# ikt-luh/Unified-Point-Cloud-Compression

Hardware: AMD Instinct MI355X
Metric: points/sec encode+decode, longdress vox10, 1 GPU; bpp & D1-PSNR parity (higher is better)
Workload: dtype f32

## Files before the change

### include/pcc_hip.h

```cpp
#ifndef PCC_HIP_H
#define PCC_HIP_H

#include <stddef.h>
#include <stdint.h>

#ifdef __cplusplus
extern "C" {
#endif

#define PCC_OK 0
#define PCC_EINVAL (-1)
#define PCC_EHIP (-2)
#define PCC_EWS (-3)

#define PCC_ACT_NONE 0
#define PCC_ACT_RELU 1
#define PCC_ACT_LEAKY 2

#define PCC_MAP_HDR_INTS 512
#define PCC_MAP_MAX_SEG 8

int pcc_version(void);
const char* pcc_last_error(void);
int pcc_device_info(int* h_cu_count, char* h_arch, int h_arch_len);
// ... 80 lines not shown
int pcc_set_in4_min_rows(int64_t rows);
int pcc_set_thin_z_min_rows(int64_t rows);
int64_t pcc_conv_packed_elems(int32_t K, int32_t cin, int32_t cout);
int pcc_conv_pack_weights(const float* W, int32_t K, int32_t cin, int32_t cout, float* packed,
                          int64_t packed_cap, void* stream);
int pcc_conv_pack_weights_ex(const float* W, int32_t K, int32_t cin, int32_t cout, int32_t transpose, int32_t flip, float* packed,
                             int64_t packed_cap, void* stream);
size_t pcc_conv_ws_bytes(int64_t n_in, int32_t K, int32_t cin, int32_t cout);
int pcc_conv_head_supported(int32_t cin, int32_t cmid);
size_t pcc_conv_head_ws_bytes(int64_t n);
int pcc_conv_head_fwd(const float* feat, int64_t n, int32_t cin, const float* packed_w0, const float* bias0 ,
                      int32_t cmid, const float* w2, const float* bias2 , const int32_t* hdr,
                      const int32_t* nbr, const int32_t* tiles, const int32_t* n_tiles, float* logits, void* ws,
                      size_t ws_bytes, void* stream);
int64_t pcc_band_tiles_cap(int64_t n, int32_t nx, int32_t nbands);
size_t pcc_band_tiles_ws_bytes(int32_t nx, int32_t nbands);
int pcc_band_tiles_build(const int64_t* keys, int64_t n, int32_t lo_x, int32_t nx, int32_t lo_y, int32_t ny, int32_t ts,
                         int32_t nbands, int32_t* tiles, int64_t tiles_cap, int32_t* n_tiles , void* ws,
                         size_t ws_bytes, void* stream);
int pcc_conv_fwd(const float* feat_in, int64_t n_in, int32_t cin, const float* packed_w,
                 const float* bias , int32_t K, int32_t cout, const int32_t* hdr,
                 const int32_t* nbr, const int32_t* rows, int64_t n_out, float* out, int32_t act,
                 float slope, void* ws, size_t ws_bytes, int32_t arith, int32_t* d_guard , void* stream);
int pcc_conv_pairs_supported(int32_t K, int32_t cin, int32_t cout);
size_t pcc_pair_plan_ws_bytes(int64_t n_out, int32_t K);
int pcc_pair_plan_rank(const int32_t* nbr, int64_t n_out, int32_t K, int32_t* pos, int32_t* pstart, int64_t* info,
                       void* ws, size_t ws_bytes, void* stream);
int pcc_pair_plan_fill(const int32_t* nbr, const int32_t* pos, const int32_t* pstart, int64_t n_out, int32_t K,
                       int64_t padded_pairs, int32_t* pair_in, int32_t* tile_k, void* stream);
int pcc_conv_fwd_pairs(const float* feat_in, int64_t n_in, int32_t cin, const float* packed_w, const float* bias,
                       int32_t K, int32_t cout, const int32_t* pair_in, const int32_t* tile_k, const int64_t* d_info,
                       int64_t padded_pairs, const int32_t* pos, int64_t n_out, float* T, float* out, int32_t act,
                       float slope, int32_t arith, int32_t* d_guard , void* stream);


int64_t pcc_convt_packed_elems(int32_t K, int32_t cin, int32_t cout);
int pcc_convt_pack_weights(const float* W, int32_t K, int32_t cin, int32_t cout, float* packed,
                           int64_t packed_cap, void* stream);
int pcc_convt_fwd(const float* feat_in, int64_t n_in, int32_t cin, const float* packed_w,
                  const float* bias , int32_t K, int32_t cout, const int32_t* hdr,
                  const int32_t* nbr, const int32_t* rows, int64_t n_out, float* T, float* out, int32_t act,
                  float slope, int32_t arith, int32_t* d_guard , void* stream);

int pcc_convt_fwd_csr(const float* feat_in, int64_t n_in, int32_t cin, const float* packed_w,
                      const float* bias , int32_t K, int32_t cout, const int32_t* first,
                      const int32_t* pair_ids, int64_t n_out, float* T, float* out, int32_t act, float slope,
                      const int32_t* ex_nbr , int32_t ex_K,
                      const float* ex_bias , int32_t arith, int32_t* d_guard , void* stream);

int pcc_convt_fwd_csr_grid(const float* feat_in, int64_t n_in, int32_t cin, const float* packed_w, const float* bias ,
                           int32_t K, int32_t cout, const int32_t* first, const int32_t* pair_ids, int64_t n_out, float* T,
                           float* out, int32_t act, float slope, const int64_t* out_keys, const uint64_t* out_bits,
                           const int32_t* out_rank, const int32_t* h_out, const float* ex_bias,
                           const int32_t* wg_end ,
                           int32_t arith, int32_t* d_guard , void* stream);
size_t pcc_thin_grid_ws_bytes(int64_t n, int32_t cout);
int pcc_conv_thin_grid_fwd(const float* feat, int64_t n, int32_t cin, const float* packed_w, const float* bias ,
                           int32_t cout, const int64_t* keys, const uint64_t* bits, const int32_t* rank, const int32_t* h_grid,
                           float* out, void* ws, size_t ws_bytes, void* stream);

int64_t pcc_gdn_packed_elems(int32_t c);
int pcc_gdn_pack(const float* beta_raw, const float* gamma_raw, int32_t c, float beta_min,
                 float* packed, int64_t packed_cap, float* beta_eff, void* stream);
int pcc_gdn_fwd(const float* x, int64_t n, int32_t c, const float* packed, const float* beta_eff,
                int32_t inverse, float* out, int32_t arith, void* stream);

// ... 161 lines not shown
```

### unified_point_cloud_compression_amd/autograd.py

```python

import torch

from . import lib as L
from . import sparse as S


GDN_FUSED_BWD = True
WGRAD_SELF = True


def _pack(w3):
    p = S.PackedConv()
    return p.get(w3.contiguous())


def _pad4(t, dim):
    r = (-t.shape[dim]) % 4
    if r == 0:
        return t
    shape = list(t.shape)
    shape[dim] = r
    return torch.cat([t, t.new_zeros(shape)], dim=dim)


def _pack_view(src3, K, cin, cout, transpose, flip):
    src3 = src3.contiguous()
    n = L.load().pcc_conv_packed_elems(K, cin, cout)
    packed = torch.empty(n, dtype=torch.float32, device=src3.device)
    L.call("pcc_conv_pack_weights_ex", L.ptr(src3), K, cin, cout, 1 if transpose else 0, 1 if flip else 0, L.ptr(packed),
           packed.numel(), L.stream())
    return packed


def _conv_view(feats, src3, transpose, flip, kmap, n_out):
    K, a, b = src3.shape
    cin, cout = (b, a) if transpose else (a, b)
    if cin % 32 == 0 and cout > 16 and feats.shape[1] == cin:
        return S.conv_forward(feats, _pack_view(src3, K, cin, cout, transpose, flip), None, K, cin, cout, kmap, n_out)
    w = torch.flip(src3, dims=[0]) if flip else src3
    return _conv_any(feats, w.permute(0, 2, 1) if transpose else w, kmap, n_out)


def _conv_any(feats, w3, kmap, n_out):
    K, cin, cout = w3.shape
    if cin % 4 != 0:
        feats, w3 = _pad4(feats, 1), _pad4(w3, 1)
        cin = w3.shape[1]
    if cin > 16 and cin % 32 != 0:
        r = (-cin) % 32
        feats = torch.cat([feats, feats.new_zeros((feats.shape[0], r))], dim=1)
        w3 = torch.cat([w3, w3.new_zeros((K, r, cout))], dim=1)
        cin += r
    if cin not in (4, 8, 16) and cin % 32 != 0:
        r = 16 - cin
        feats = torch.cat([feats, feats.new_zeros((feats.shape[0], r))], dim=1)
        w3 = torch.cat([w3, w3.new_zeros((K, r, cout))], dim=1)
        cin = 16
    return S.conv_forward(feats, _pack(w3), None, K, cin, cout, kmap, n_out)


class SparseConvFn(torch.autograd.Function):

    @staticmethod
    def forward(ctx, feats, kernel, bias, module, in_set, out_set, kmap, act, slope):
        K, cin, cout = module.kernel_volume, module.in_channels, module.out_channels
        packed = module._packed.get(kernel, tag_from=module.kernel)
        feats = feats.contiguous()
        if isinstance(kmap, tuple):
            out = S.convt_forward_csr(feats, packed, bias, K, cin, cout, kmap, out_set.n, act, slope)
        elif module.TRANSPOSED:
            out = S.convt_forward(feats, packed, bias, K, cin, cout, kmap, out_set.n, act, slope)
        else:
            out = S.conv_forward(feats, packed, bias, K, cin, cout, kmap, out_set.n, act, slope)
        ctx.save_for_backward(feats, kernel, out if act != L.ACT_NONE else None)
        ctx.meta = (module, in_set, out_set, kmap, act, slope, bias is not None)
        return out

    @staticmethod
    def backward(ctx, g):
        feats, kernel, out = ctx.saved_tensors
        module, in_set, out_set, kmap, act, slope, has_bias = ctx.meta
        K, cin, cout = module.kernel_volume, module.in_channels, module.out_channels
        g = g.contiguous()
        if act == L.ACT_RELU:
            g = g * (out > 0)
        elif act == L.ACT_LEAKY:
            g = torch.where(out > 0, g, g * slope)
        w3 = kernel.detach() if kernel.dim() == 3 else kernel.detach().unsqueeze(0)
        g_feats = g_kernel = g_bias = None
        if has_bias and ctx.needs_input_grad[2]:
            g_bias = g.sum(dim=0, keepdim=True)
        if module.TRANSPOSED:
            if not isinstance(kmap, tuple):
                raise L.PccError("backward of the transposed conv needs the CSR pair lists (sparse.USE_CSR)")
            dT = S.convt_scatter_rows(g, kmap, feats.shape[0] * K, cout).view(feats.shape[0], K * cout)
            if ctx.needs_input_grad[1]:
                gw = S.conv_wgrad(feats, dT, 1, cin, K * cout, None)[0]
                g_kernel = gw.view(cin, K, cout).permute(1, 0, 2).contiguous()
            if ctx.needs_input_grad[0]:
                wt = w3.permute(0, 2, 1).reshape(1, K * cout, cin)
                g_feats = _conv_any(dT, wt, None, feats.shape[0])
        else:
            if ctx.needs_input_grad[1]:
                if (WGRAD_SELF and in_set is out_set and kmap is not None and kmap.rows is None and module.stride == 1
                        and g.shape[0] == feats.shape[0] and L.load().pcc_conv_wgrad_self_supported(K, cin, cout)):
                    g_kernel = S.conv_wgrad_self(feats, g, K, cin, kmap, cout)
# ... 212 lines not shown
```

### unified_point_cloud_compression_amd/csrc/pcc_conv.hip

```cpp
#include <vector>

#include "pcc_common.h"

typedef float f32x16 __attribute__((ext_vector_type(16)));

static constexpr int LDS_LD = 36;
static constexpr int MAXK = 128;
static constexpr int MAXK_T = 512;

enum { MODE_CONV = 0, MODE_GDN = 1, MODE_IGDN = 2 };
#ifdef PCC_DBG_BUILD
#define PCC_DBG_ON(a, bit) (((a).dbg & (bit)) != 0)
#else
#define PCC_DBG_ON(a, bit) false
#endif
__device__ inline float act1(float v, int act, float slope);

struct ConvArgs {
  const float* feat;
  const float* wp;
  const float* bias;
  const int* hdr;
  const int* nbr;
  const int* rows;
  float* out;
  long long n_out;
  long long n_in;
  long long wp_elems;
  const int* pair_in = nullptr;
  const int* tile_k = nullptr;
  const long long* n_tiles = nullptr;
  const unsigned char* featb = nullptr;
  int ksplit = 1;
  float* part = nullptr;
  int dbg = 0;
  int nt = 0;
  bool wh_ok = false;
  const unsigned char* feath = nullptr;
  const float* frow_inv = nullptr;
  int arith = PCC_ARITH_H3;
  int* guard = nullptr;
  float guard_lim = 0.f;
  int cin, cout, cout_pad;
  int cb_log2;
  int ppo;
  int act;
  float slope;
};

__host__ __device__ inline int bn_for(int cout) { return cout >= 128 ? 128 : (cout > 32 ? 64 : 32); }

static constexpr unsigned BUF_OOB = 0xFFFF0000u;
static constexpr long long BUF_MAX_BYTES = 0xFFFE0000ll;

template <int WM, int WN, int TM, int TN, int MODE, bool BUF>
__global__ void __launch_bounds__(256) k_conv_mfma(ConvArgs a) {
  constexpr int BM = WM * TM * 32;
  constexpr int BN = WN * TN * 32;
  static_assert(WM * WN == 4, "4 waves per workgroup");
  __shared__ __attribute__((aligned(16))) float As[BM * LDS_LD];
  __shared__ __attribute__((aligned(16))) float Bs[BN * LDS_LD];
  __shared__ unsigned char act_flag[MAXK];
  __shared__ unsigned char act_list[MAXK];
  __shared__ unsigned char act_kid[MAXK];
  __shared__ int s_nact;

  const int tid = threadIdx.x, lane = tid & 63, w = tid >> 6;

  const int cpx = gridDim.x >> 3;
  const int wid = (blockIdx.x & 7) * cpx + (blockIdx.x >> 3);
  const int gy = a.cout_pad / BN;
  int tile_id = wid / gy;
  int colblock = (wid - tile_id * gy) * BN;
  if (a.hdr == nullptr && a.pair_in == nullptr && gy > 8) {
    const int g = wid / (8 * gy), rem = wid - g * 8 * gy;
    colblock = (rem >> 3) * BN;
    tile_id = g * 8 + (rem & 7);
  }

  int pos0, npos, k_count, koff_begin;
  long long seg_pos_count;
  const int* seg_nbr = nullptr;
  const bool pair_mode = (a.pair_in != nullptr);
  bool identity = (a.hdr == nullptr) && !pair_mode;
  if (pair_mode) {
    if (tile_id >= *a.n_tiles) return;
    pos0 = tile_id * BM; npos = BM; k_count = 1; koff_begin = 0; seg_pos_count = 0;
    seg_nbr = a.pair_in + pos0;
  } else if (identity) {
    const long long p0 = (long long)tile_id * BM;
    if (p0 >= a.n_out) return;
    pos0 = (int)p0;
    npos = (int)min((long long)BM, a.n_out - p0);
    k_count = 1; koff_begin = 0; seg_pos_count = a.n_out;
  } else {
    const int nseg = a.hdr[HDR_NSEG];
    int tile = tile_id, s = 0;
    bool found = false;
    int pb = 0, pc = 0;
    for (; s < nseg; ++s) {
      const int* sg = a.hdr + HDR_SEG0 + s * SEG_WORDS;
      pb = sg[SEG_POS_BEGIN]; pc = sg[SEG_POS_COUNT];
      const int tiles = (pc + BM - 1) / BM;
      if (tile < tiles) { found = true; break; }
      tile -= tiles;
    }
    if (!found) return;
    const int* sg = a.hdr + HDR_SEG0 + s * SEG_WORDS;
    k_count = sg[SEG_K_COUNT];
    koff_begin = sg[SEG_KOFF_BEGIN];
    const long long nb = ((long long)(unsigned)sg[SEG_NBR_LO]) | ((long long)sg[SEG_NBR_HI] << 32);
    seg_nbr = a.nbr + nb;
    seg_pos_count = pc;
    const int local0 = tile * BM;
    pos0 = pb + local0;
    npos = min(BM, pc - local0);
    seg_nbr += local0;
  }

// ... 422 lines not shown
  constexpr int BM = WM * TM * 32;
  constexpr int BN = WN * TN * 32;
  static_assert(WM * WN == 4, "4 waves per workgroup");
  static_assert(BN <= 128 && BM <= 128, "one feature row and one weight row per thread (pair)");
  constexpr int LDU = 13;
  __shared__ __attribute__((aligned(16))) uint4 As[BM * LDU];
  __shared__ __attribute__((aligned(16))) uint4 Bs[BN * LDU];
  __shared__ unsigned char act_flag[MAXK];
  __shared__ unsigned char act_list[MAXK];
  __shared__ unsigned char act_kid[MAXK];
  __shared__ int s_nact;

  const int tid = threadIdx.x, lane = tid & 63, w = tid >> 6;
  const int cpx = gridDim.x >> 3;
  int wid = (blockIdx.x & 7) * cpx + (blockIdx.x >> 3);
  const int ks_id = wid % a.ksplit;
  wid /= a.ksplit;
  const int gy = a.cout_pad / BN;
  int tile_id = wid / gy;
  int colblock = (wid - tile_id * gy) * BN;
  if (a.hdr == nullptr && a.pair_in == nullptr && gy > 8) {
    const int g = wid / (8 * gy), rem = wid - g * 8 * gy;
    colblock = (rem >> 3) * BN;
    tile_id = g * 8 + (rem & 7);
  }

  int pos0, npos, k_count, koff_begin;
  long long seg_pos_count;
  const int* seg_nbr = nullptr;
  const bool pair_mode = (a.pair_in != nullptr);
  const bool identity = (a.hdr == nullptr) && !pair_mode;
  if (pair_mode) {
    if (tile_id >= *a.n_tiles) return;
    pos0 = tile_id * BM; npos = BM; k_count = 1; koff_begin = 0; seg_pos_count = 0;
    seg_nbr = a.pair_in + pos0;
  } else if (identity) {
    const long long p0 = (long long)tile_id * BM;
    if (p0 >= a.n_out) return;
    pos0 = (int)p0;
    npos = (int)min((long long)BM, a.n_out - p0);
    k_count = 1; koff_begin = 0; seg_pos_count = a.n_out;
  } else {
    const int nseg = a.hdr[HDR_NSEG];
    int tile = tile_id, sgi = 0;
    bool found = false;
    int pb = 0, pc = 0;
    for (; sgi < nseg; ++sgi) {
      const int* sg = a.hdr + HDR_SEG0 + sgi * SEG_WORDS;
      pb = sg[SEG_POS_BEGIN]; pc = sg[SEG_POS_COUNT];
      const int tiles = (pc + BM - 1) / BM;
      if (tile < tiles) { found = true; break; }
      tile -= tiles;
    }
    if (!found) return;
    const int* sg = a.hdr + HDR_SEG0 + sgi * SEG_WORDS;
    k_count = sg[SEG_K_COUNT];
    koff_begin = sg[SEG_KOFF_BEGIN];
    const long long nb = ((long long)(unsigned)sg[SEG_NBR_LO]) | ((long long)sg[SEG_NBR_HI] << 32);
    seg_nbr = a.nbr + nb;
    seg_pos_count = pc;
    const int local0 = tile * BM;
    pos0 = pb + local0;
    npos = min(BM, pc - local0);
    seg_nbr += local0;
  }

// ... 740 lines not shown
#pragma unroll
      for (int e1 = 0; e1 < 4; ++e1) {
        const int e = e4 * 4 + e1;
        const int rrow = i * 32 + e1 + 8 * e4;
        const unsigned so = (unsigned)rrow * ncol * 4u;
#pragma unroll
        for (int j = 0; j < TN; ++j) {
          const float v = acc[i][j][e] * (rr[e1] * cs[j]);
          if (full && nt) {
            __builtin_amdgcn_raw_buffer_store_b32(__float_as_uint(v), rsO, vO + (unsigned)j * 128u, (int)so, 2);
          } else if (full) {
            __builtin_amdgcn_raw_buffer_store_b32(__float_as_uint(v), rsO, vO + (unsigned)j * 128u, (int)so, 0);
          } else {
            const unsigned off = (rrow < row_lim && j * 32 < col_lim) ? vO + (unsigned)j * 128u + so : BUF_OOB;
            __builtin_amdgcn_raw_buffer_store_b32(__float_as_uint(v), rsO, off, 0, 0);
          }
        }
      }
    }
  if (a.guard && guard_mr * guard_mc * (8.f * (float)a.cin) > a.guard_lim) atomicOr(a.guard, 1);
}

template <int NCH>
__global__ void __launch_bounds__(256, 3) k_pair_h2(ConvArgs a) {
  constexpr int BM = 128, BN = 128, LDU = 9;
  constexpr unsigned ROWB = NCH * 128u;
  __shared__ __attribute__((aligned(16))) uint4 As[BM * LDU];
  __shared__ __attribute__((aligned(16))) uint4 Bs[BN * LDU];
  __shared__ __attribute__((aligned(16))) float rs[BM];
  const int tid = threadIdx.x, lane = tid & 63, w = tid >> 6;
  const int cpx = gridDim.x >> 3;
  const int wid = (blockIdx.x & 7) * cpx + (blockIdx.x >> 3);
  const int gy = a.cout_pad / BN;
  const int tile_id = wid / gy;
  const int colblock = (wid - tile_id * gy) * BN;
  if (tile_id >= *a.n_tiles) return;
  const long long p0 = (long long)tile_id * BM;
  const int kid = a.tile_k[tile_id];

  const __amdgpu_buffer_rsrc_t rsA = __builtin_amdgcn_make_buffer_rsrc(
      const_cast<unsigned char*>(a.feath), (short)0, (int)(unsigned)((size_t)a.n_in * ROWB), 0x00020000);
  const float* const wplanes = a.wp + a.wp_elems + bf_plane_elems(a.wp_elems);
  const unsigned char* wb = reinterpret_cast<const unsigned char*>(wplanes) + ((size_t)kid * NCH * a.cout_pad + colblock) * 128u;
  const float* const cinv = wplanes + a.wp_elems + (size_t)kid * a.cout_pad;
  const unsigned b_stride = (unsigned)a.cout_pad * 128u;
  const __amdgpu_buffer_rsrc_t rsB = __builtin_amdgcn_make_buffer_rsrc(
      const_cast<unsigned char*>(wb), (short)0, (int)((NCH - 1) * b_stride + BN * 128u), 0x00020000);

  unsigned vA[4], ld[4];
#pragma unroll
  for (int j = 0; j < 4; ++j) {
    const unsigned u = (unsigned)(j * 256 + tid), row = u >> 3, wu = u & 7u;
    const int g = a.pair_in[p0 + row];
    vA[j] = g >= 0 ? (unsigned)g * ROWB + wu * 16u : BUF_OOB;
    ld[j] = row * LDU + wu;
  }
  const unsigned vB = (unsigned)tid * 16u;

  uint4 av[4], bv[4];
  auto issue = [&](int cbi) {
#pragma unroll
    for (int j = 0; j < 4; ++j)
      av[j] = __builtin_bit_cast(uint4, __builtin_amdgcn_raw_buffer_load_b128(rsA, vA[j] == BUF_OOB ? BUF_OOB : vA[j] + (unsigned)cbi * 128u, 0, 0));
#pragma unroll
    for (int j = 0; j < 4; ++j)
      bv[j] = __builtin_bit_cast(uint4, __builtin_amdgcn_raw_buffer_load_b128(rsB, vB, (int)((unsigned)cbi * b_stride + (unsigned)j * 4096u), 0));
  };

  f32x16 acc[2][2];
// ... 1234 lines not shown
  long long run = 0;
  for (int k = 0; k < K; ++k) {
    pstart[k] = (int)run;
    run += (cnt[k] + PAIR_BM - 1) / PAIR_BM * PAIR_BM;
  }
  pstart[K] = (int)run;
  info[0] = run; info[1] = run / PAIR_BM; info[2] = total;
}

__global__ void k_pair_pos(const int* __restrict__ nbr, const int* __restrict__ g, const int* __restrict__ pstart,
                           long long n_out, int K, int* __restrict__ pos) {
  const long long o = (long long)blockIdx.x * blockDim.x + threadIdx.x;
  const int k = blockIdx.y;
  if (o >= n_out) return;
  const long long e = (long long)k * n_out + o;
  pos[e] = nbr[e] >= 0 ? pstart[k] + (g[e] - g[(long long)k * n_out]) : -1;
}

__global__ void k_pair_fill(const int* __restrict__ nbr, const int* __restrict__ pos, long long n,
                            int* __restrict__ pair_in) {
  const long long e = (long long)blockIdx.x * blockDim.x + threadIdx.x;
  if (e < n && pos[e] >= 0) pair_in[pos[e]] = nbr[e];
}

__global__ void k_pair_tile_k(const int* __restrict__ pstart, int K, long long tiles, int* __restrict__ tile_k) {
  const long long t = (long long)blockIdx.x * blockDim.x + threadIdx.x;
  if (t >= tiles) return;
  const long long p = t * PAIR_BM;
  int lo = 0, hi = K;
  while (hi - lo > 1) { const int mid = (lo + hi) >> 1; if (pstart[mid] <= p) lo = mid; else hi = mid; }
  tile_k[t] = lo;
}

extern "C" int pcc_conv_pairs_supported(int32_t K, int32_t cin, int32_t cout) {
  return (K >= 1 && K <= MAXK && conv_kind(K, cin, cout) == KIND_MFMA && cout % 4 == 0) ? 1 : 0;
}

extern "C" size_t pcc_pair_plan_ws_bytes(int64_t n_out, int32_t K) {
  const int64_t n = n_out * K;
  return 2 * pcc_align_up((size_t)n * 4) + pcc_scan_ws_bytes(n) + 1024;
}

extern "C" int pcc_pair_plan_rank(const int32_t* nbr, int64_t n_out, int32_t K, int32_t* pos, int32_t* pstart,
                                  int64_t* info, void* ws, size_t ws_bytes, void* stream) {
  hipStream_t s = (hipStream_t)stream;
  PCC_REQUIRE(nbr && pos && pstart && info && ws && n_out > 0 && K >= 1 && K <= MAXK, "pcc_pair_plan_rank: bad arguments");
  const int64_t n = n_out * K;
  PCC_REQUIRE(n + (int64_t)K * PAIR_BM < (1ll << 31), "pcc_pair_plan_rank: too many map slots");
  if (ws_bytes < pcc_pair_plan_ws_bytes(n_out, K)) { pcc_set_error("pcc_pair_plan_rank: workspace too small"); return PCC_EWS; }
  char* p = (char*)ws;
  int* f = (int*)p;  p += pcc_align_up((size_t)n * 4);
  int* g = (int*)p;  p += pcc_align_up((size_t)n * 4);
  k_pair_flags<<<(unsigned)pcc_cdiv(n, 256), 256, 0, s>>>(nbr, n, f);
  PCC_LAUNCH_CHECK();
  PCC_TRY(pcc_scan_exclusive_i32(f, g, n, p, ws_bytes - (size_t)(p - (char*)ws), s));
  k_pair_starts<<<1, 128, 0, s>>>(g, nbr, n_out, K, pstart, (long long*)info);
  PCC_LAUNCH_CHECK();
  k_pair_pos<<<dim3((unsigned)pcc_cdiv(n_out, 256), (unsigned)K), 256, 0, s>>>(nbr, g, pstart, n_out, K, pos);
  PCC_LAUNCH_CHECK();
  return PCC_OK;
}

extern "C" int pcc_pair_plan_fill(const int32_t* nbr, const int32_t* pos, const int32_t* pstart, int64_t n_out, int32_t K,
                                  int64_t padded_pairs, int32_t* pair_in, int32_t* tile_k, void* stream) {
  hipStream_t s = (hipStream_t)stream;
  PCC_REQUIRE(nbr && pos && pstart && pair_in && tile_k && padded_pairs % PAIR_BM == 0, "pcc_pair_plan_fill: bad arguments");
  if (padded_pairs == 0) return PCC_OK;
  PCC_CHECK_HIP(hipMemsetAsync(pair_in, 0xFF, (size_t)padded_pairs * 4, s));
  const int64_t n = n_out * K;
  k_pair_fill<<<(unsigned)pcc_cdiv(n, 256), 256, 0, s>>>(nbr, pos, n, pair_in);
  PCC_LAUNCH_CHECK();
  const int64_t tiles = padded_pairs / PAIR_BM;
  k_pair_tile_k<<<(unsigned)pcc_cdiv(tiles, 256), 256, 0, s>>>(pstart, K, tiles, tile_k);
  PCC_LAUNCH_CHECK();
  return PCC_OK;
}

struct PairReduceArgs {
  const float* T; const float* bias; const int* pos; float* out; long long n_out; int K, cout, act; float slope; int lpr_log2;
};

__global__ void __launch_bounds__(256) k_pair_reduce(PairReduceArgs a) {
  constexpr int JB = 5;
  const int lane = threadIdx.x & 63;
  const int lpr = 1 << a.lpr_log2;
  const int rpw = 64 >> a.lpr_log2;
  const long long o = ((long long)blockIdx.x * 4 + (threadIdx.x >> 6)) * rpw + (lane >> a.lpr_log2);
  const int cl = lane & (lpr - 1);
  if (o >= a.n_out) return;
  const int cvec = a.cout / 4;
  for (int cv = cl; cv < cvec; cv += lpr) {
    float4 acc = make_float4(0.f, 0.f, 0.f, 0.f);
    for (int k0 = 0; k0 < a.K; k0 += JB) {
      int pr[JB];
#pragma unroll
      for (int u = 0; u < JB; ++u) pr[u] = (k0 + u < a.K) ? a.pos[(long long)(k0 + u) * a.n_out + o] : -1;
      float4 x[JB];
#pragma unroll
      for (int u = 0; u < JB; ++u) {
        x[u] = make_float4(0.f, 0.f, 0.f, 0.f);
        if (pr[u] >= 0) x[u] = reinterpret_cast<const float4*>(a.T + (long long)pr[u] * a.cout)[cv];
      }
#pragma unroll
      for (int u = 0; u < JB; ++u) { acc.x += x[u].x; acc.y += x[u].y; acc.z += x[u].z; acc.w += x[u].w; }
    }
    if (a.bias) {
      const float4 b = reinterpret_cast<const float4*>(a.bias)[cv];
      acc.x += b.x; acc.y += b.y; acc.z += b.z; acc.w += b.w;
    }
    acc.x = act1(acc.x, a.act, a.slope); acc.y = act1(acc.y, a.act, a.slope);
    acc.z = act1(acc.z, a.act, a.slope); acc.w = act1(acc.w, a.act, a.slope);
    reinterpret_cast<float4*>(a.out + o * a.cout)[cv] = acc;
  }
}

extern "C" int pcc_conv_fwd_pairs(const float* feat_in, int64_t n_in, int32_t cin, const float* packed_w,
                                  const float* bias, int32_t K, int32_t cout, const int32_t* pair_in,
                                  const int32_t* tile_k, const int64_t* d_info, int64_t padded_pairs,
                                  const int32_t* pos, int64_t n_out, float* T, float* out, int32_t act, float slope,
                                  int32_t arith, int32_t* d_guard, void* stream) {
  hipStream_t s = (hipStream_t)stream;
  if (n_out <= 0) return PCC_OK;
  PCC_REQUIRE(feat_in && packed_w && pair_in && tile_k && d_info && pos && T && out, "pcc_conv_fwd_pairs: NULL array");
  PCC_REQUIRE(conv_kind(K, cin, cout) == KIND_MFMA && cout % 4 == 0, "pcc_conv_fwd_pairs: shape cin=%d cout=%d not on the MFMA path", cin, cout);
  PCC_REQUIRE(padded_pairs % PAIR_BM == 0 && padded_pairs < (1ll << 31), "pcc_conv_fwd_pairs: bad pair count");
  PCC_REQUIRE(act >= 0 && act <= 2, "pcc_conv_fwd_pairs: bad activation");
  if (padded_pairs > 0) {
    ConvArgs a;
    a.feat = feat_in; a.wp = packed_w; a.bias = nullptr; a.hdr = nullptr; a.nbr = nullptr; a.rows = nullptr; a.out = T;
    a.n_out = padded_pairs; a.cin = cin; a.cout = cout; a.cout_pad = cout_pad_for(cout);
    a.n_in = n_in; a.wp_elems = (long long)K * cin * a.cout_pad;
    a.cb_log2 = cb_log2_for(cin); a.ppo = cin >> a.cb_log2; a.act = 0; a.slope = 0.f;
    a.pair_in = pair_in; a.tile_k = tile_k; a.n_tiles = (const long long*)d_info + 1;
    PCC_TRY(set_arith(a, arith, d_guard, "pcc_conv_fwd_pairs"));
    hipEvent_t e0, e1;
    if (g_prof_on) PCC_TRY(prof_event(&e0, s));
    const int bn = bn_for(cout);
    const long long gy = a.cout_pad / bn;
    const dim3 grid((unsigned)((padded_pairs / PAIR_BM * gy + 7) / 8 * 8));
    const bool buf = g_mfma_buf && n_in * cin * 4 <= BUF_MAX_BYTES && a.wp_elems * 4 <= BUF_MAX_BYTES;
    const bool split = split_ok(a);
    const bool pair_h = split && a.arith == PCC_ARITH_H3 && conv_has_h(K, cin, cout) && (size_t)n_in * cin * 4 <= (size_t)BUF_MAX_BYTES &&
                        (a.ppo == 1 || a.ppo == 2 || a.ppo == 4 || a.ppo == 6 || a.ppo == 8);
    prof_note(pair_h ? PCC_FORM_PAIR_H2 : split ? PCC_FORM_PAIR_BF : PCC_FORM_CONV_F32, 0.0, 0.0);
    if (pair_h) {
      PCC_TRY(make_planes_h(a, s));
      switch (a.ppo) {
        case 1: k_pair_h2<1><<<grid, 256, 0, s>>>(a); break;
        case 2: k_pair_h2<2><<<grid, 256, 0, s>>>(a); break;
        case 4: k_pair_h2<4><<<grid, 256, 0, s>>>(a); break;
        case 6: k_pair_h2<6><<<grid, 256, 0, s>>>(a); break;
        default: k_pair_h2<8><<<grid, 256, 0, s>>>(a); break;
      }
    } else if (split) PCC_TRY(make_planes(a, false, s));
    if (pair_h) {}
    else if (bn == 128) { if (split) k_conv_mfma_bf<2, 2, 2, 2, MODE_CONV><<<grid, 256, 0, s>>>(a); else if (buf) k_conv_mfma<2, 2, 2, 2, MODE_CONV, true><<<grid, 256, 0, s>>>(a); else k_conv_mfma<2, 2, 2, 2, MODE_CONV, false><<<grid, 256, 0, s>>>(a); }
    else if (bn == 64) { if (split) k_conv_mfma_bf<2, 2, 2, 1, MODE_CONV><<<grid, 256, 0, s>>>(a); else if (buf) k_conv_mfma<2, 2, 2, 1, MODE_CONV, true><<<grid, 256, 0, s>>>(a); else k_conv_mfma<2, 2, 2, 1, MODE_CONV, false><<<grid, 256, 0, s>>>(a); }
    else { if (split) k_conv_mfma_bf<4, 1, 1, 1, MODE_CONV><<<grid, 256, 0, s>>>(a); else if (buf) k_conv_mfma<4, 1, 1, 1, MODE_CONV, true><<<grid, 256, 0, s>>>(a); else k_conv_mfma<4, 1, 1, 1, MODE_CONV, false><<<grid, 256, 0, s>>>(a); }
    PCC_LAUNCH_CHECK();
    if (g_prof_on) {
      PCC_TRY(prof_event(&e1, s));
      prof_push();
    }
  }
  PairReduceArgs r;
  r.T = T; r.bias = bias; r.pos = pos; r.out = out; r.n_out = n_out; r.K = K; r.cout = cout; r.act = act; r.slope = slope;
  int l = 0;
  while ((1 << l) < cout / 4 && l < 6) ++l;
  r.lpr_log2 = l;
  const int64_t waves = pcc_cdiv(n_out, 64 >> l);
  k_pair_reduce<<<(unsigned)pcc_cdiv(waves, 4), 256, 0, s>>>(r);
  PCC_LAUNCH_CHECK();
  return PCC_OK;
}

static constexpr int CK_T = 256, CK_I = 8, CK_B = CK_T * CK_I;

__global__ void __launch_bounds__(CK_T) k_csr_khist(const int* __restrict__ pair_ids, const int* __restrict__ d_P, int K,
                                                    int nb, int* __restrict__ hist) {
  __shared__ int h[MAXK];
  for (int i = threadIdx.x; i < K; i += CK_T) h[i] = 0;
  __syncthreads();
  const int P = *d_P;
  const long long base = (long long)blockIdx.x * CK_B;
#pragma unroll
  for (int r = 0; r < CK_I; ++r) {
    const long long t = base + r * CK_T + threadIdx.x;
    if (t < P) atomicAdd(&h[pair_ids[t] % K], 1);
  }
  __syncthreads();
  for (int i = threadIdx.x; i < K; i += CK_T) hist[(long long)i * nb + blockIdx.x] = h[i];
}

__global__ void __launch_bounds__(128) k_csr_kstarts(const int* __restrict__ off, const int* __restrict__ d_P, int K, int nb,
                                                     int* __restrict__ pstart, long long* __restrict__ info) {
  __shared__ long long cnt[MAXK];
  const long long total = *d_P;
  for (int k = threadIdx.x; k < K; k += blockDim.x) {
    const long long b = off[(long long)k * nb];
    const long long e = (k + 1 < K) ? off[(long long)(k + 1) * nb] : total;
    cnt[k] = e - b;
  }
  __syncthreads();
  if (threadIdx.x != 0) return;
  long long run = 0;
  for (int k = 0; k < K; ++k) {
// ... 868 lines not shown
```

### unified_point_cloud_compression_amd/lib.py

```python
import ctypes as C
import os
import threading

import torch

_HERE = os.path.dirname(os.path.abspath(__file__))
LIB_PATH = os.path.join(_HERE, "libpcc_hip.so")

MAP_HDR_INTS = 512
FORM_NAMES = ("other", "k_gemm_h2", "k_gemm_bf2", "k_pair_h2", "pair_bf", "k_conv_mfma_bf", "k_conv_mfma", "k_conv_wave16",
              "k_convt_gather_csr")
MAP_MAX_SEG = 8
ACT_NONE, ACT_RELU, ACT_LEAKY = 0, 1, 2

_p = C.c_void_p
_i32, _i64, _u64, _f32, _sz = C.c_int32, C.c_int64, C.c_uint64, C.c_float, C.c_size_t

SIGNATURES = {
    "pcc_version": (C.c_int, []),
    "pcc_last_error": (C.c_char_p, []),
    "pcc_device_info": (C.c_int, [C.POINTER(C.c_int), C.c_char_p, C.c_int]),
    "pcc_coords_bounds": (C.c_int, [_p, _i32, _i64, _p, _p]),
    "pcc_rows_gather": (C.c_int, [_p, _p, _i64, _i32, _p, _p]),
    "pcc_keys_pack_i32": (C.c_int, [_p, _i64, _p, _p]),
# ... 88 lines not shown
    "pcc_topk_prune_keys": (C.c_int, [_p, _i64, C.POINTER(_i64), C.POINTER(_i64), _i32, _p, _p, _p, _p, _sz, _p]),
    "pcc_prune_ws_bytes": (_sz, [_i64]),
    "pcc_prune_rows": (C.c_int, [_p, _i64, _p, _p, _i32, _p, _p, _p, _p, _sz, _p]),
    "pcc_lookup_gather": (C.c_int, [_p, _i64, _p, _i32, _p, _i64, _p, _p]),
    "pcc_lookup_rows": (C.c_int, [_p, _i64, _p, _i64, _p, _p]),
    "pcc_gauss_encode": (C.c_int, [_p, _p, _p, _p, _i64, _i32, _p, _i32, _p, _p, _p, _p]),
    "pcc_gauss_decode": (C.c_int, [_p, _p, _p, _p, _i64, _i32, _p, _i32, _p, _p, _p]),
    "pcc_eb_encode": (C.c_int, [_p, _i64, _i32, _p, _p, _p, _p, _p, _p]),
    "pcc_eb_lik_fwd": (C.c_int, [_p, _i64, _i32, _p, _p, _p]),
    "pcc_eb_lik_bwd": (C.c_int, [_p, _p, _i64, _i32, _p, _p, _p, _p]),
    "pcc_pmf_to_quantized_cdf": (C.c_int, [_p, _i32, _i32, _p]),
    "pcc_rans_max_bytes": (_i64, [_i64]),
    "pcc_rans_encode_host": (C.c_int, [_p, _p, _i64, _p, _i32, _p, _p, _p, _i64, C.POINTER(_i64)]),
    "pcc_rans_decode_host": (C.c_int, [_p, _i64, _p, _i64, _p, _i32, _p, _p, _p]),
    "pcc_rans_container_max_bytes": (_i64, [_i64, _i32]),
    "pcc_rans_streams_ws_bytes": (_sz, [_i64, _i32]),
    "pcc_rans_build_enc_table": (C.c_int, [_p, _i32, _i32, _p, _p]),
    "pcc_rans_stream_symbols": (_i64, [_i64, _i32, _i32, _i32]),
    "pcc_rans_estimate_bits": (C.c_int, [_p, _p, _i64, _i32, _p, _i32, _p, _p, _p, _p]),
    "pcc_rans_encode_streams": (C.c_int, [_p, _p, _i64, _i32, _i32, _i32, _p, _i32, _p, _p, _p, _p, _p, _p, _sz, _p]),
    "pcc_rans_dec_table_bytes": (_i64, [_i32, _p]),
    "pcc_rans_build_dec_table": (C.c_int, [_p, _i32, _i32, _p, _p]),
    "pcc_rans_decode_streams": (C.c_int, [_p, _i64, _p, _i64, _i32, _i32, _i32, _p, _i32, _p, _p, _p, _i64, _p, _p, _p]),
    "pcc_rans_decode_streams_form": (C.c_int, [_p, _i64, _p, _i64, _i32, _i32, _i32, _p, _i32, _p, _p, _p, _i64, _p, _p, _p, _i32]),
    "pcc_octree_max_bytes": (_i64, [_i64, _i32]),
    "pcc_octree_encode_host": (C.c_int, [_p, _i64, _i32, _p, _i64, C.POINTER(_i64)]),
    "pcc_octree_decode_host": (C.c_int, [_p, _i64, _p, _i64, C.POINTER(_i64), C.POINTER(_i32)]),
    "pcc_conv_pairs_supported": (C.c_int, [_i32, _i32, _i32]),
    "pcc_pair_plan_ws_bytes": (_sz, [_i64, _i32]),
    "pcc_pair_plan_rank": (C.c_int, [_p, _i64, _i32, _p, _p, _p, _p, _sz, _p]),
    "pcc_pair_plan_fill": (C.c_int, [_p, _p, _p, _i64, _i32, _i64, _p, _p, _p]),
    "pcc_conv_fwd_pairs": (C.c_int, [_p, _i64, _i32, _p, _p, _i32, _i32, _p, _p, _p, _i64, _p, _i64, _p, _p, _i32,
                                     C.c_float, _i32, _p, _p]),
    "pcc_nn_sorted_x": (C.c_int, [_p, _i64, _p, _i64, _p, _p, _p]),
    "pcc_normals_grid": (C.c_int, [_p, _i64, _p, C.POINTER(_i32), _i32, _p, _p, _p]),
    "pcc_cube_keys": (C.c_int, [_p, _i64, _i32, _p, _p, _p, _p]),
    "pcc_cube_regroup": (C.c_int, [_p, _p, _p, _i64, _p, _p, _p]),
    "pcc_aug_gray_sums": (C.c_int, [_p, _i64, _p, _p, _i32, _p, _p, _i32, _p, _p, _p]),
    "pcc_aug_batch": (C.c_int, [_p, _p, _i64, _p, _p, _i32, _p, _p, _i32, _p, _p, _p, _i64, _p, _p]),
    "pcc_prof_enable": (C.c_int, [_i32]),
    "pcc_prof_collect": (C.c_int, [C.POINTER(C.c_double), C.POINTER(_i64)]),
    "pcc_prof_sequence": (_i64, [C.POINTER(_i32), _i64]),
    "pcc_prof_collect_forms": (C.c_int, [C.POINTER(C.c_double), C.POINTER(_i64), C.POINTER(C.c_double), C.POINTER(C.c_double)]),
}

_lib = None


class PccError(RuntimeError):
    pass


def load():
    global _lib
    if _lib is not None:
        return _lib
    if not os.path.exists(LIB_PATH):
        raise PccError(
            f"{LIB_PATH} is missing: the HIP extension is not built. Run `python -c 'import __graft_entry__ as g; "
            f"g.build()'` (or `make -C unified_point_cloud_compression_amd/csrc`). There is no CPU fallback.")
    lib = C.CDLL(LIB_PATH)
    for name, (res, args) in SIGNATURES.items():
        fn = getattr(lib, name)
        fn.restype = res
        fn.argtypes = args
    _lib = lib
# ... 159 lines not shown
```

### unified_point_cloud_compression_amd/sparse.py

```python
import ctypes as C

import itertools
import weakref

import torch

from . import lib as L

BIAS = 1 << 15


def _field_mask(lo, hi):
    a, b = lo + BIAS, hi + BIAS
    return (1 << (a ^ b).bit_length()) - 1


class Bounds:

    def __init__(self, bmax, lo, hi):
        self.bmax, self.lo, self.hi = int(bmax), tuple(int(v) for v in lo), tuple(int(v) for v in hi)
        if min(self.lo) < -BIAS + 64 or max(self.hi) >= BIAS - 64 or self.bmax >= (1 << 15):
            raise L.PccError(f"coordinates out of the 16-bit key range: lo={self.lo} hi={self.hi} batch={self.bmax}")

    def bit_mask(self):
# ... 13 lines not shown

class KernelMap:

    def pairs(self):
        if self._pairs is None:
            self._pairs = int(self.d_pairs.item()) if self.d_pairs is not None else -1
        return self._pairs

    def pair_plan_begin(self):
        if hasattr(self, "_plan"):
            return _ready(self._plan)
        if hasattr(self, "_plan_pending"):
            return self._plan_pending
        if not (self.rows is None and not self.transposed and self.n_out > 0 and self.K * self.n_out + self.K * 128 < (1 << 31)):
            self._plan = None
            return _ready(None)
        dev = self.hdr.device
        lib = L.load()
        pos = torch.empty(self.K * self.n_out, dtype=torch.int32, device=dev)
        pstart = torch.empty(self.K + 1, dtype=torch.int32, device=dev)
        info = L.counter(3)
        ws = L.workspace(lib.pcc_pair_plan_ws_bytes(self.n_out, self.K), dev)
        L.call("pcc_pair_plan_rank", L.ptr(self.nbr), self.n_out, self.K, L.ptr(pos), L.ptr(pstart), L.ptr(info),
               L.ptr(ws), ws.numel(), L.stream())

        def finish(v):
            padded, _, pairs = (int(x) for x in v)
            if self._pairs is None:
                self._pairs = pairs
            self._plan = None
            if pairs <= PAIR_MAX_DENSITY * self.K * self.n_out:
                pair_in = torch.empty(max(padded, 1), dtype=torch.int32, device=dev)
                tile_k = torch.empty(max(padded // 128, 1), dtype=torch.int32, device=dev)
                L.call("pcc_pair_plan_fill", L.ptr(self.nbr), L.ptr(pos), L.ptr(pstart), self.n_out, self.K, padded,
                       L.ptr(pair_in), L.ptr(tile_k), L.stream())
                self._plan = (pos, pair_in, tile_k, info, padded)
            del self._plan_pending
            return self._plan
        self._plan_pending = Pending(info, finish)
        return self._plan_pending

    def pair_plan(self):
        if not hasattr(self, "_plan"):
            resolve(self.pair_plan_begin())
        return self._plan

    def dense(self):
        out = torch.empty((self.K, self.n_out), dtype=torch.int32, device=self.hdr.device)
        if self.n_out:
            L.call("pcc_map_to_dense", L.ptr(self.hdr), L.ptr(self.nbr), L.ptr(self.rows), self.n_out, self.K,
                   L.ptr(out), L.stream())
        return out


PAIR_MIN_K = 64
PAIR_MAX_DENSITY = 0.5
PAIR_MIN_CIN = 64
COUNT_PAIRS = False
MORTON_MIN_ROWS = 1 << 62
USE_CSR = True
CANON_BY_GRID = True
EXPAND_BY_GRID = True
STRIDE_BY_GRID = True
USE_GRID = True
GRID_MAX_BYTES = 8 << 30
BAND_TILES = True
BAND_MIN_ROWS = 1 << 20
BAND_COUNT = 16
# ... 480 lines not shown
class PackedConv:

    def __init__(self, transposed=False):
        self.tag = None
        self.packed = None
        self.transposed = transposed

    def get(self, kernel, state_dict_order=False, tag_from=None):
        w = kernel.detach()
        src = tag_from if tag_from is not None else kernel
        tag = (src.data_ptr(), src._version, tuple(w.shape), str(w.device),
               WEIGHT_OFFSET_ORDER if (state_dict_order or tag_from is not None) else "")
        if tag != self.tag:
            w3 = w if w.dim() == 3 else w.unsqueeze(0)
            perm = weight_offset_perm(w3.shape[0], w3.device) if state_dict_order else None
            if perm is not None:
                w3 = w3[perm]
            w3 = w3.to(torch.float32).contiguous()
            K, cin, cout = w3.shape
            pre = "pcc_convt" if self.transposed else "pcc_conv"
            n = getattr(L.load(), pre + "_packed_elems")(K, cin, cout)
            if n <= 0:
                raise L.PccError(f"unsupported convolution shape K={K} cin={cin} cout={cout}")
            self.packed = torch.empty(n, dtype=torch.float32, device=w.device)
            L.call(pre + "_pack_weights", L.ptr(w3), K, cin, cout, L.ptr(self.packed), self.packed.numel(), L.stream())
            self.tag = tag
        return self.packed


def wants_pairs(K, cin, cout):
    return bool(K >= PAIR_MIN_K and cin >= PAIR_MIN_CIN and L.load().pcc_conv_pairs_supported(K, cin, cout))


def conv_forward(feats, packed_w, bias, K, cin, cout, kmap, n_out, act=L.ACT_NONE, slope=0.01):
    feats = feats.contiguous()
    out = torch.empty((n_out, cout), dtype=torch.float32, device=feats.device)
    if n_out == 0:
        return out
    b = bias.detach().reshape(-1).contiguous() if bias is not None else None
    if kmap is not None and wants_pairs(K, cin, cout):
        plan = kmap.pair_plan()
        if plan is not None:
            pos, pair_in, tile_k, info, padded = plan
            T = L.workspace(max(padded, 1) * cout * 4, feats.device)
            L.call("pcc_conv_fwd_pairs", L.ptr(feats), feats.shape[0], cin, L.ptr(packed_w), L.ptr(b), K, cout,
                   L.ptr(pair_in), L.ptr(tile_k), L.ptr(info), padded, L.ptr(pos), n_out, L.ptr(T), L.ptr(out), act,
                   float(slope), *L.arith_args(feats.device), L.stream())
            return out
    ws = L.workspace(L.load().pcc_conv_ws_bytes(feats.shape[0], K, cin, cout), feats.device)
    L.call("pcc_conv_fwd", L.ptr(feats), feats.shape[0], cin, L.ptr(packed_w), L.ptr(b), K, cout,
           L.ptr(kmap.hdr) if kmap is not None else None, L.ptr(kmap.nbr) if kmap is not None else None,
           L.ptr(kmap.rows) if kmap is not None else None, n_out, L.ptr(out), act, float(slope), L.ptr(ws),
           ws.numel(), *L.arith_args(feats.device), L.stream())
    return out


def conv_head_forward(feats, packed_w0, bias0, cmid, w2, bias2, cset, kmap):
    feats = feats.contiguous()
    n, cin = feats.shape
    out = torch.empty((n, 1), dtype=torch.float32, device=feats.device)
    if n == 0:
        return out
    bands = cset.band_tiles()
    ws = L.workspace(L.load().pcc_conv_head_ws_bytes(n), feats.device)
    b0 = bias0.detach().reshape(-1).contiguous() if bias0 is not None else None
    b2 = bias2.detach().reshape(-1).contiguous() if bias2 is not None else None
    L.call("pcc_conv_head_fwd", L.ptr(feats), n, cin, L.ptr(packed_w0), L.ptr(b0), cmid, L.ptr(w2), L.ptr(b2),
           L.ptr(kmap.hdr), L.ptr(kmap.nbr), L.ptr(bands[0]) if bands else None, L.ptr(bands[1]) if bands else None,
           L.ptr(out), L.ptr(ws), ws.numel(), L.stream())
    return out


def convt_forward(feats, packed_w, bias, K, cin, cout, kmap, n_out, act=L.ACT_NONE, slope=0.01):
    feats = feats.contiguous()
    n_in = feats.shape[0]
    out = torch.empty((n_out, cout), dtype=torch.float32, device=feats.device)
    if n_out == 0 or n_in == 0:
        return out
    T = torch.empty(n_in * K * cout, dtype=torch.float32, device=feats.device)
    b = bias.detach().reshape(-1).contiguous() if bias is not None else None
# ... 272 lines not shown
```

Before: 54.49 million.

## Reorder pair-conv tiles by kernel-offset group and output position for cache locality

Adds a tile permutation to the pair-based sparse convolution. Tiles are grouped by kernel offset modulo the kernel side length and ordered by output position, so concurrently running workgroups touch nearby input features and weights. The permutation is built once per kernel map by a new ranking kernel, and the conv kernels remap tile ids through it. The intent is better L2 reuse of gathered features, at the cost of an extra plan-build kernel, an extra indirection per tile, and possibly worse weight reuse within a single offset.

```diff
diff --git a/include/pcc_hip.h b/include/pcc_hip.h
--- a/include/pcc_hip.h
+++ b/include/pcc_hip.h
@@ -136,6 +136,15 @@
                        int32_t K, int32_t cout, const int32_t* pair_in, const int32_t* tile_k, const int64_t* d_info,
                        int64_t padded_pairs, const int32_t* pos, int64_t n_out, float* T, float* out, int32_t act,
                        float slope, int32_t arith, int32_t* d_guard , void* stream);
+int pcc_pair_order_groups(int32_t K);
+int pcc_pair_plan_fill_ordered(const int32_t* nbr, const int32_t* pos, const int32_t* pstart, int64_t n_out, int32_t K,
+                               int64_t padded_pairs, int32_t* pair_in, int32_t* tile_k, int32_t* tile_o,
+                               int32_t* tile_order, void* stream);
+int pcc_conv_fwd_pairs_ordered(const float* feat_in, int64_t n_in, int32_t cin, const float* packed_w, const float* bias,
+                               int32_t K, int32_t cout, const int32_t* pair_in, const int32_t* tile_k,
+                               const int32_t* tile_order , const int64_t* d_info, int64_t padded_pairs,
+                               const int32_t* pos, int64_t n_out, float* T, float* out, int32_t act, float slope,
+                               int32_t arith, int32_t* d_guard , void* stream);
 
 
 int64_t pcc_convt_packed_elems(int32_t K, int32_t cin, int32_t cout);
diff --git a/unified_point_cloud_compression_amd/autograd.py b/unified_point_cloud_compression_amd/autograd.py
--- a/unified_point_cloud_compression_amd/autograd.py
+++ b/unified_point_cloud_compression_amd/autograd.py
@@ -36,7 +36,8 @@
     K, a, b = src3.shape
     cin, cout = (b, a) if transpose else (a, b)
     if cin % 32 == 0 and cout > 16 and feats.shape[1] == cin:
-        return S.conv_forward(feats, _pack_view(src3, K, cin, cout, transpose, flip), None, K, cin, cout, kmap, n_out)
+        return S.conv_forward(feats, _pack_view(src3, K, cin, cout, transpose, flip), None, K, cin, cout, kmap, n_out,
+                              tile_order=False)
     w = torch.flip(src3, dims=[0]) if flip else src3
     return _conv_any(feats, w.permute(0, 2, 1) if transpose else w, kmap, n_out)
 
@@ -56,7 +57,7 @@
         feats = torch.cat([feats, feats.new_zeros((feats.shape[0], r))], dim=1)
         w3 = torch.cat([w3, w3.new_zeros((K, r, cout))], dim=1)
         cin = 16
-    return S.conv_forward(feats, _pack(w3), None, K, cin, cout, kmap, n_out)
+    return S.conv_forward(feats, _pack(w3), None, K, cin, cout, kmap, n_out, tile_order=False)
 
 
 class SparseConvFn(torch.autograd.Function):
@@ -71,7 +72,8 @@
         elif module.TRANSPOSED:
             out = S.convt_forward(feats, packed, bias, K, cin, cout, kmap, out_set.n, act, slope)
         else:
-            out = S.conv_forward(feats, packed, bias, K, cin, cout, kmap, out_set.n, act, slope)
+            out = S.conv_forward(feats, packed, bias, K, cin, cout, kmap, out_set.n, act, slope,
+                                 tile_order=False)
         ctx.save_for_backward(feats, kernel, out if act != L.ACT_NONE else None)
         ctx.meta = (module, in_set, out_set, kmap, act, slope, bias is not None)
         return out
diff --git a/unified_point_cloud_compression_amd/csrc/pcc_conv.hip b/unified_point_cloud_compression_amd/csrc/pcc_conv.hip
--- a/unified_point_cloud_compression_amd/csrc/pcc_conv.hip
+++ b/unified_point_cloud_compression_amd/csrc/pcc_conv.hip
@@ -29,6 +29,7 @@
   long long wp_elems;
   const int* pair_in = nullptr;
   const int* tile_k = nullptr;
+  const int* tile_order = nullptr;
   const long long* n_tiles = nullptr;
   const unsigned char* featb = nullptr;
   int ksplit = 1;
@@ -85,6 +86,7 @@
   bool identity = (a.hdr == nullptr) && !pair_mode;
   if (pair_mode) {
     if (tile_id >= *a.n_tiles) return;
+    if (a.tile_order) tile_id = a.tile_order[tile_id];
     pos0 = tile_id * BM; npos = BM; k_count = 1; koff_begin = 0; seg_pos_count = 0;
     seg_nbr = a.pair_in + pos0;
   } else if (identity) {
@@ -573,6 +575,7 @@
   const bool identity = (a.hdr == nullptr) && !pair_mode;
   if (pair_mode) {
     if (tile_id >= *a.n_tiles) return;
+    if (a.tile_order) tile_id = a.tile_order[tile_id];
     pos0 = tile_id * BM; npos = BM; k_count = 1; koff_begin = 0; seg_pos_count = 0;
     seg_nbr = a.pair_in + pos0;
   } else if (identity) {
@@ -1379,9 +1382,10 @@
   const int cpx = gridDim.x >> 3;
   const int wid = (blockIdx.x & 7) * cpx + (blockIdx.x >> 3);
   const int gy = a.cout_pad / BN;
-  const int tile_id = wid / gy;
-  const int colblock = (wid - tile_id * gy) * BN;
-  if (tile_id >= *a.n_tiles) return;
+  const int slot = wid / gy;
+  const int colblock = (wid - slot * gy) * BN;
+  if (slot >= *a.n_tiles) return;
+  const int tile_id = a.tile_order ? a.tile_order[slot] : slot;
   const long long p0 = (long long)tile_id * BM;
   const int kid = a.tile_k[tile_id];
 
@@ -2682,6 +2686,52 @@
   tile_k[t] = lo;
 }
 
+#ifndef PAIR_ORDER_GROUPS
+#define PAIR_ORDER_GROUPS 0
+#endif
+
+__global__ void k_pair_fill_o(const int* __restrict__ nbr, const int* __restrict__ pos, long long n, long long n_out,
+                              int* __restrict__ pair_in, int* __restrict__ tile_o) {
+  const long long e = (long long)blockIdx.x * blockDim.x + threadIdx.x;
+  if (e >= n) return;
+  const int p = pos[e];
+  if (p < 0) return;
+  pair_in[p] = nbr[e];
+  if ((p & (PAIR_BM - 1)) == 0) tile_o[p / PAIR_BM] = (int)(e % n_out);
+}
+
+__global__ void __launch_bounds__(256) k_pair_tile_order(const int* __restrict__ pstart, const int* __restrict__ tile_o, int K,
+                                                         int gm, long long tiles, int* __restrict__ tile_order) {
+  __shared__ int tstart[MAXK + 1];
+  for (int k = threadIdx.x; k <= K; k += blockDim.x) tstart[k] = pstart[k] / PAIR_BM;
+  __syncthreads();
+  const long long t = (long long)blockIdx.x * blockDim.x + threadIdx.x;
+  if (t >= tiles) return;
+  if (gm == 0) { tile_order[t] = (int)t; return; }
+  int lo = 0, hi = K;
+  while (hi - lo > 1) { const int mid = (lo + hi) >> 1; if (tstart[mid] <= t) lo = mid; else hi = mid; }
+  const int k = lo, g = k % gm, o = tile_o[t];
+  long long rank = 0;
+  for (int k2 = 0; k2 < K; ++k2) {
+    const int g2 = k2 % gm, b = tstart[k2], e = tstart[k2 + 1];
+    if (g2 < g) { rank += e - b; continue; }
+    if (g2 > g || b == e) continue;
+    if (k2 == k) { rank += t - b; continue; }
+    const int lim = k2 < k ? o + 1 : o;
+    int l = b, h = e;
+    while (l < h) { const int mid = (l + h) >> 1; if (tile_o[mid] < lim) l = mid + 1; else h = mid; }
+    rank += l - b;
+  }
+  tile_order[rank] = (int)t;
+}
+
+static int pair_order_gm(int K) {
+  int ks = 1;
+  while (ks * ks * ks < K) ++ks;
+  if (ks * ks * ks != K) return 0;
+  return PAIR_ORDER_GROUPS == 0 ? ks : PAIR_ORDER_GROUPS == 1 ? 1 : ks * ks;
+}
+
 extern "C" int pcc_conv_pairs_supported(int32_t K, int32_t cin, int32_t cout) {
   return (K >= 1 && K <= MAXK && conv_kind(K, cin, cout) == KIND_MFMA && cout % 4 == 0) ? 1 : 0;
 }
@@ -2711,20 +2761,40 @@
   return PCC_OK;
 }
 
-extern "C" int pcc_pair_plan_fill(const int32_t* nbr, const int32_t* pos, const int32_t* pstart, int64_t n_out, int32_t K,
-                                  int64_t padded_pairs, int32_t* pair_in, int32_t* tile_k, void* stream) {
-  hipStream_t s = (hipStream_t)stream;
-  PCC_REQUIRE(nbr && pos && pstart && pair_in && tile_k && padded_pairs % PAIR_BM == 0, "pcc_pair_plan_fill: bad arguments");
+static int pair_plan_fill(const int32_t* nbr, const int32_t* pos, const int32_t* pstart, int64_t n_out, int32_t K,
+                          int64_t padded_pairs, int32_t* pair_in, int32_t* tile_k, int32_t* tile_o, int32_t* tile_order,
+                          hipStream_t s) {
   if (padded_pairs == 0) return PCC_OK;
   PCC_CHECK_HIP(hipMemsetAsync(pair_in, 0xFF, (size_t)padded_pairs * 4, s));
   const int64_t n = n_out * K;
-  k_pair_fill<<<(unsigned)pcc_cdiv(n, 256), 256, 0, s>>>(nbr, pos, n, pair_in);
+  if (tile_order) k_pair_fill_o<<<(unsigned)pcc_cdiv(n, 256), 256, 0, s>>>(nbr, pos, n, n_out, pair_in, tile_o);
+  else k_pair_fill<<<(unsigned)pcc_cdiv(n, 256), 256, 0, s>>>(nbr, pos, n, pair_in);
   PCC_LAUNCH_CHECK();
   const int64_t tiles = padded_pairs / PAIR_BM;
   k_pair_tile_k<<<(unsigned)pcc_cdiv(tiles, 256), 256, 0, s>>>(pstart, K, tiles, tile_k);
   PCC_LAUNCH_CHECK();
+  if (tile_order) {
+    k_pair_tile_order<<<(unsigned)pcc_cdiv(tiles, 256), 256, 0, s>>>(pstart, tile_o, K, pair_order_gm(K), tiles, tile_order);
+    PCC_LAUNCH_CHECK();
+  }
   return PCC_OK;
 }
+
+extern "C" int pcc_pair_plan_fill(const int32_t* nbr, const int32_t* pos, const int32_t* pstart, int64_t n_out, int32_t K,
+                                  int64_t padded_pairs, int32_t* pair_in, int32_t* tile_k, void* stream) {
+  PCC_REQUIRE(nbr && pos && pstart && pair_in && tile_k && padded_pairs % PAIR_BM == 0, "pcc_pair_plan_fill: bad arguments");
+  return pair_plan_fill(nbr, pos, pstart, n_out, K, padded_pairs, pair_in, tile_k, nullptr, nullptr, (hipStream_t)stream);
+}
+
+extern "C" int pcc_pair_plan_fill_ordered(const int32_t* nbr, const int32_t* pos, const int32_t* pstart, int64_t n_out,
+                                          int32_t K, int64_t padded_pairs, int32_t* pair_in, int32_t* tile_k,
+                                          int32_t* tile_o, int32_t* tile_order, void* stream) {
+  PCC_REQUIRE(nbr && pos && pstart && pair_in && tile_k && tile_o && tile_order && padded_pairs % PAIR_BM == 0 && n_out > 0 &&
+              K >= 1 && K <= MAXK, "pcc_pair_plan_fill_ordered: bad arguments");
+  return pair_plan_fill(nbr, pos, pstart, n_out, K, padded_pairs, pair_in, tile_k, tile_o, tile_order, (hipStream_t)stream);
+}
+
+extern "C" int pcc_pair_order_groups(int32_t K) { return pair_order_gm(K); }
 
 struct PairReduceArgs {
   const float* T; const float* bias; const int* pos; float* out; long long n_out; int K, cout, act; float slope; int lpr_log2;
@@ -2764,11 +2834,11 @@
   }
 }
 
-extern "C" int pcc_conv_fwd_pairs(const float* feat_in, int64_t n_in, int32_t cin, const float* packed_w,
-                                  const float* bias, int32_t K, int32_t cout, const int32_t* pair_in,
-                                  const int32_t* tile_k, const int64_t* d_info, int64_t padded_pairs,
-                                  const int32_t* pos, int64_t n_out, float* T, float* out, int32_t act, float slope,
-                                  int32_t arith, int32_t* d_guard, void* stream) {
+static int conv_fwd_pairs(const float* feat_in, int64_t n_in, int32_t cin, const float* packed_w,
+                          const float* bias, int32_t K, int32_t cout, const int32_t* pair_in,
+                          const int32_t* tile_k, const int32_t* tile_order, const int64_t* d_info, int64_t padded_pairs,
+                          const int32_t* pos, int64_t n_out, float* T, float* out, int32_t act, float slope,
+                          int32_t arith, int32_t* d_guard, void* stream) {
   hipStream_t s = (hipStream_t)stream;
   if (n_out <= 0) return PCC_OK;
   PCC_REQUIRE(feat_in && packed_w && pair_in && tile_k && d_info && pos && T && out, "pcc_conv_fwd_pairs: NULL array");
@@ -2781,7 +2851,7 @@
     a.n_out = padded_pairs; a.cin = cin; a.cout = cout; a.cout_pad = cout_pad_for(cout);
     a.n_in = n_in; a.wp_elems = (long long)K * cin * a.cout_pad;
     a.cb_log2 = cb_log2_for(cin); a.ppo = cin >> a.cb_log2; a.act = 0; a.slope = 0.f;
-    a.pair_in = pair_in; a.tile_k = tile_k; a.n_tiles = (const long long*)d_info + 1;
+    a.pair_in = pair_in; a.tile_k = tile_k; a.tile_order = tile_order; a.n_tiles = (const long long*)d_info + 1;
     PCC_TRY(set_arith(a, arith, d_guard, "pcc_conv_fwd_pairs"));
     hipEvent_t e0, e1;
     if (g_prof_on) PCC_TRY(prof_event(&e0, s));
@@ -2822,6 +2892,24 @@
   k_pair_reduce<<<(unsigned)pcc_cdiv(waves, 4), 256, 0, s>>>(r);
   PCC_LAUNCH_CHECK();
   return PCC_OK;
+}
+
+extern "C" int pcc_conv_fwd_pairs(const float* feat_in, int64_t n_in, int32_t cin, const float* packed_w,
+                                  const float* bias, int32_t K, int32_t cout, const int32_t* pair_in,
+                                  const int32_t* tile_k, const int64_t* d_info, int64_t padded_pairs,
+                                  const int32_t* pos, int64_t n_out, float* T, float* out, int32_t act, float slope,
+                                  int32_t arith, int32_t* d_guard, void* stream) {
+  return conv_fwd_pairs(feat_in, n_in, cin, packed_w, bias, K, cout, pair_in, tile_k, nullptr, d_info, padded_pairs, pos, n_out,
+                        T, out, act, slope, arith, d_guard, stream);
+}
+
+extern "C" int pcc_conv_fwd_pairs_ordered(const float* feat_in, int64_t n_in, int32_t cin, const float* packed_w,
+                                          const float* bias, int32_t K, int32_t cout, const int32_t* pair_in,
+                                          const int32_t* tile_k, const int32_t* tile_order, const int64_t* d_info,
+                                          int64_t padded_pairs, const int32_t* pos, int64_t n_out, float* T, float* out,
+                                          int32_t act, float slope, int32_t arith, int32_t* d_guard, void* stream) {
+  return conv_fwd_pairs(feat_in, n_in, cin, packed_w, bias, K, cout, pair_in, tile_k, tile_order, d_info, padded_pairs, pos,
+                        n_out, T, out, act, slope, arith, d_guard, stream);
 }
 
 static constexpr int CK_T = 256, CK_I = 8, CK_B = CK_T * CK_I;
diff --git a/unified_point_cloud_compression_amd/lib.py b/unified_point_cloud_compression_amd/lib.py
--- a/unified_point_cloud_compression_amd/lib.py
+++ b/unified_point_cloud_compression_amd/lib.py
@@ -144,6 +144,10 @@
     "pcc_pair_plan_fill": (C.c_int, [_p, _p, _p, _i64, _i32, _i64, _p, _p, _p]),
     "pcc_conv_fwd_pairs": (C.c_int, [_p, _i64, _i32, _p, _p, _i32, _i32, _p, _p, _p, _i64, _p, _i64, _p, _p, _i32,
                                      C.c_float, _i32, _p, _p]),
+    "pcc_pair_order_groups": (C.c_int, [_i32]),
+    "pcc_pair_plan_fill_ordered": (C.c_int, [_p, _p, _p, _i64, _i32, _i64, _p, _p, _p, _p, _p]),
+    "pcc_conv_fwd_pairs_ordered": (C.c_int, [_p, _i64, _i32, _p, _p, _i32, _i32, _p, _p, _p, _p, _i64, _p, _i64, _p, _p, _i32,
+                                             C.c_float, _i32, _p, _p]),
     "pcc_nn_sorted_x": (C.c_int, [_p, _i64, _p, _i64, _p, _p, _p]),
     "pcc_normals_grid": (C.c_int, [_p, _i64, _p, C.POINTER(_i32), _i32, _p, _p, _p]),
     "pcc_cube_keys": (C.c_int, [_p, _i64, _i32, _p, _p, _p, _p]),
diff --git a/unified_point_cloud_compression_amd/sparse.py b/unified_point_cloud_compression_amd/sparse.py
--- a/unified_point_cloud_compression_amd/sparse.py
+++ b/unified_point_cloud_compression_amd/sparse.py
@@ -69,8 +69,10 @@
             if pairs <= PAIR_MAX_DENSITY * self.K * self.n_out:
                 pair_in = torch.empty(max(padded, 1), dtype=torch.int32, device=dev)
                 tile_k = torch.empty(max(padded // 128, 1), dtype=torch.int32, device=dev)
-                L.call("pcc_pair_plan_fill", L.ptr(self.nbr), L.ptr(pos), L.ptr(pstart), self.n_out, self.K, padded,
-                       L.ptr(pair_in), L.ptr(tile_k), L.stream())
+                tile_o = torch.empty_like(tile_k)
+                self._plan_order = torch.empty_like(tile_k)
+                L.call("pcc_pair_plan_fill_ordered", L.ptr(self.nbr), L.ptr(pos), L.ptr(pstart), self.n_out, self.K, padded,
+                       L.ptr(pair_in), L.ptr(tile_k), L.ptr(tile_o), L.ptr(self._plan_order), L.stream())
                 self._plan = (pos, pair_in, tile_k, info, padded)
             del self._plan_pending
             return self._plan
@@ -617,7 +619,7 @@
     return bool(K >= PAIR_MIN_K and cin >= PAIR_MIN_CIN and L.load().pcc_conv_pairs_supported(K, cin, cout))
 
 
-def conv_forward(feats, packed_w, bias, K, cin, cout, kmap, n_out, act=L.ACT_NONE, slope=0.01):
+def conv_forward(feats, packed_w, bias, K, cin, cout, kmap, n_out, act=L.ACT_NONE, slope=0.01, tile_order=True):
     feats = feats.contiguous()
     out = torch.empty((n_out, cout), dtype=torch.float32, device=feats.device)
     if n_out == 0:
@@ -628,9 +630,10 @@
         if plan is not None:
             pos, pair_in, tile_k, info, padded = plan
             T = L.workspace(max(padded, 1) * cout * 4, feats.device)
-            L.call("pcc_conv_fwd_pairs", L.ptr(feats), feats.shape[0], cin, L.ptr(packed_w), L.ptr(b), K, cout,
-                   L.ptr(pair_in), L.ptr(tile_k), L.ptr(info), padded, L.ptr(pos), n_out, L.ptr(T), L.ptr(out), act,
-                   float(slope), *L.arith_args(feats.device), L.stream())
+            order = getattr(kmap, "_plan_order", None) if tile_order else None
+            L.call("pcc_conv_fwd_pairs_ordered", L.ptr(feats), feats.shape[0], cin, L.ptr(packed_w), L.ptr(b), K, cout,
+                   L.ptr(pair_in), L.ptr(tile_k), L.ptr(order), L.ptr(info), padded, L.ptr(pos), n_out, L.ptr(T),
+                   L.ptr(out), act, float(slope), *L.arith_args(feats.device), L.stream())
             return out
     ws = L.workspace(L.load().pcc_conv_ws_bytes(feats.shape[0], K, cin, cout), feats.device)
     L.call("pcc_conv_fwd", L.ptr(feats), feats.shape[0], cin, L.ptr(packed_w), L.ptr(b), K, cout,
```

Result: no change. 54.25 million (-0.5%).
